# mariaalfaroc/omr_a2s_multimodal_transformer

Measured on AMD Instinct MI355X. Metric: training samples/sec, higher is better.
Workload: dtype bf16; 1 GPU; C2: image encoder (CNN) + 6-layer d_model=256 kern decoder, fwd+bwd+Adam, dropout on, teacher-forcing noise on; one sample = one score image + its token sequence; per_gpu_batch=32, global_batch=32, image=256x2048x1, seq_len=512, layers=6, d_model=256, vocab=6997, parallelism=dp1

## Files before the change

### omr_a2s_multimodal_transformer_amd/csrc/conv3x3_mfma.h

```cpp
#pragma once
#include <type_traits>

#include "omr_common.h"
#include "launch_setup.h"

namespace omr_conv {

constexpr int NORM_MAX = 128;
constexpr int TW = 32;

template <int G, typename F, typename LoadFn, typename StoreFn>
__device__ __forceinline__ void staged_walk(int pix0, int npix, int DP, int il0, int jl0, int di, int dj, int IW, LoadFn load, StoreFn store) {
    int il = il0, jl = jl0;
    for (int base = pix0; base < npix; base += G * DP) {
        F v[G];
        int pix = base;
#pragma unroll
        for (int g = 0; g < G; ++g) {
            if (pix < npix) v[g] = load(il, jl);
            jl += dj; il += di;
            if (jl >= IW) { jl -= IW; ++il; }
            pix += DP;
        }
        pix = base;
#pragma unroll
        for (int g = 0; g < G; ++g) {
            if (pix < npix) store(pix, v[g]);
            pix += DP;
        }
    }
}

__host__ __device__ constexpr bool conv_subpix(int SH, int SW, int DH, int DW, int RPW) { return DH == 2 && DW == 2 && SH == 1 && SW == 1 && RPW == 2; }
__host__ __device__ constexpr int conv_halo_h(int TH, int SH, bool subpix) { return subpix ? ((TH - 1) * SH + 3 + 1) / 2 : (TH - 1) * SH + 3; }
__host__ __device__ constexpr int conv_halo_w(int SW, bool subpix) { return subpix ? ((TW - 1) * SW + 3) / 2 : (TW - 1) * SW + 3; }

struct ConvArgs {
    const void* x; const void* w; const float* bias; void* y;
    const float* mean; const float* rstd;
    const void* mask; float mask_scale;
    int B, Hr, Wr, CIN, Ho, Wo, COUT;
    int sh, sw, dh, dw, relu, tiles_w, tiles_h;
    uint32_t drop_thresh; float drop_scale; uint64_t drop_seed; int drop_channel;
    int stat_mode; double* stat_ws; const void* stat_x; const float* stat_mean; const float* stat_rstd; int stat_slots;
    int stat_relu; float stat_relu_scale;
};

template <typename T, int NT, int RPW, int CK, int SH, int SW, int DH, int DW, bool SINGLE, int EPI>
__global__ __launch_bounds__(256, (SINGLE && NT == 32) ? ((CK == 16 && EPI != 2) ? 4 : 3) : 2) void conv3x3_mfma_kernel(ConvArgs a) {
    typedef typename Frag<T>::type F;
    typedef __attribute__((ext_vector_type(4))) T T4;
    constexpr int VEC = Frag<T>::N;
    constexpr int CKP = CK + VEC;
    constexpr int NB = NT / 32;
    constexpr int TH = 4 * RPW;
    constexpr bool SUBPIX = conv_subpix(SH, SW, DH, DW, RPW);
    constexpr int IH = conv_halo_h(TH, SH, SUBPIX), IW = conv_halo_w(SW, SUBPIX), NPIX = IH * IW;
    constexpr int CPP = CK / VEC;
    constexpr int OP = NT + VEC;
    constexpr int XS_ELEMS = (SINGLE && TH * TW * OP > NPIX * CKP) ? TH * TW * OP : NPIX * CKP;
    extern __shared__ __attribute__((aligned(16))) unsigned char smem_raw[];
    T* Xs = reinterpret_cast<T*>(smem_raw);
    T* Os = Xs;
    T* Ws = Xs + XS_ELEMS;

    const int tid = threadIdx.x, lane = tid & 63, wave = tid >> 6;
    const int n0 = blockIdx.y * NT;
    const int Hv = (a.Hr - 1) * DH + 1, Wv = (a.Wr - 1) * DW + 1;
    const T* W = (const T*)a.w;
    constexpr bool single = SINGLE;
    const int frow = lane & 31, fk = (lane >> 5) * VEC, hsel = 4 * (lane >> 5);
    const int sp_rp = wave >> 1;
    const int sp_row = (wave & 1) * 4 + sp_rp + 2 * (frow >> 4), sp_col = 2 * (frow & 15);

    auto stage_weights = [&](int c0) {
        constexpr int NCH = NT * 9 * CPP, ROUNDS = (NCH + 255) / 256, GB = 4;
#pragma unroll
        for (int r0 = 0; r0 < ROUNDS; r0 += GB) {
            F v[GB];
#pragma unroll
            for (int g = 0; g < GB; ++g) {
                const int c = tid + (r0 + g) * 256, row = c / CPP, kc = (c % CPP) * VEC, n = n0 + row / 9;
                v[g] = frag_zero<T>();
                if (r0 + g < ROUNDS && c < NCH && n < a.COUT) v[g] = *reinterpret_cast<const F*>(W + ((long)n * 9 + row % 9) * a.CIN + c0 + kc);
            }
#pragma unroll
            for (int g = 0; g < GB; ++g) {
                const int c = tid + (r0 + g) * 256, row = c / CPP, kc = (c % CPP) * VEC;
                if (r0 + g < ROUNDS && c < NCH) *reinterpret_cast<F*>(Ws + (long)row * CKP + kc) = v[g];
            }
        }
    };

    __shared__ __attribute__((aligned(16))) float sbias[NT];
    for (int i = tid; i < NT; i += 256) sbias[i] = (a.bias && n0 + i < a.COUT) ? a.bias[n0 + i] : 0.f;

    __shared__ __attribute__((aligned(16))) float snorm[2 * NORM_MAX];
    if (a.mean)
        for (int i = tid; i < a.CIN; i += 256) {
            snorm[i] = a.mean[(long)blockIdx.z * a.CIN + i];
            snorm[NORM_MAX + i] = a.rstd[(long)blockIdx.z * a.CIN + i];
        }

    if (single) stage_weights(0);

    constexpr int CPO = NT / VEC;
    constexpr int NSV = EPI ? VEC : 1;
    float ssum[NSV], ssq[NSV], smu[EPI == 2 ? VEC : 1], srs[EPI == 2 ? VEC : 1];
#pragma unroll
    for (int e = 0; e < NSV; ++e) ssum[e] = ssq[e] = 0.f;
#pragma unroll
    for (int e = 0; e < (EPI == 2 ? VEC : 1); ++e) { smu[e] = 0.f; srs[e] = 1.f; }
    constexpr bool FWD = EPI == 1 || EPI == 3, DROP = EPI == 3;
    const bool stat1 = FWD && a.stat_mode == 1, stat2 = EPI == 2 && (a.stat_mode == 2 || a.stat_mode == 4);
    const bool apply5 = EPI == 2 && a.stat_mode == 5, store_y = a.stat_mode != 4;
    auto flush_stats = [&](int bimg) {
        if constexpr (EPI != 0) {
            constexpr int NGRP = 256 / CPO;
            constexpr int RP = NT + 1;
            static_assert((size_t)NGRP * RP * sizeof(float) <= ((size_t)XS_ELEMS + (size_t)NT * 9 * CKP) * sizeof(T), "reduction scratch fits in the (dead) halo + weight tiles");
            float* red = reinterpret_cast<float*>(smem_raw);
#pragma unroll
            for (int k = 0; k < 2; ++k) {
                __syncthreads();
                const int kcs = (tid % CPO) * VEC, grp = tid / CPO;
#pragma unroll
                for (int e = 0; e < NSV; ++e) red[grp * RP + kcs + e] = k ? ssq[e] : ssum[e];
                __syncthreads();
                for (int i = tid; i < NT; i += 256) {
                    const int n = n0 + i;
                    double acc2 = 0.0;
                    for (int g = 0; g < NGRP; ++g) acc2 += (double)red[g * RP + i];
                    if (n < a.COUT) {
                        a.stat_ws[(((long)bimg * a.stat_slots + blockIdx.x) * a.COUT + n) * 2 + k] = acc2;
                        if (blockIdx.x == 0)
                            for (int sl = gridDim.x; sl < a.stat_slots; ++sl) a.stat_ws[(((long)bimg * a.stat_slots + sl) * a.COUT + n) * 2 + k] = 0.0;
                    }
                }
            }
        }
    };

    const int tiles_per_img = a.tiles_h * a.tiles_w;
    const int b = blockIdx.z;
    if constexpr (EPI == 2) {
        if (stat2 || apply5) {
            const double* compact = a.stat_ws + (long)a.B * a.stat_slots * a.COUT * 2;
            const double inv_hw = 1.0 / ((double)a.Ho * a.Wo);
#pragma unroll
            for (int e = 0; e < VEC; ++e) {
                const int n = n0 + (tid % CPO) * VEC + e;
                smu[e] = n < a.COUT ? a.stat_mean[(long)b * a.COUT + n] : 0.f;
                srs[e] = n < a.COUT ? a.stat_rstd[(long)b * a.COUT + n] : 1.f;
                if (apply5) {
                    ssum[e] = n < a.COUT ? (float)(compact[((long)b * a.COUT + n) * 2] * inv_hw) : 0.f;
                    ssq[e] = n < a.COUT ? (float)(compact[((long)b * a.COUT + n) * 2 + 1] * inv_hw) : 0.f;
                }
            }
        }
    }
    uint32_t ckeep[NB];
#pragma unroll
    for (int j = 0; j < NB; ++j) ckeep[j] = 0xffffu;
    if constexpr (DROP) {
        if (a.drop_thresh && a.drop_channel) {
#pragma unroll
            for (int j = 0; j < NB; ++j) {
                ckeep[j] = 0;
#pragma unroll
                for (int r = 0; r < 16; r += 2) {
                    const uint32_t hsh = drop_pair_bits(a.drop_seed, ((uint64_t)b * a.COUT + n0 + j * 32 + 8 * (r >> 2) + hsel + (r & 3)) >> 1);
                    ckeep[j] |= (uint32_t)((hsh & 0xffffu) >= a.drop_thresh) << r | (uint32_t)((hsh >> 16) >= a.drop_thresh) << (r + 1);
                }
            }
        }
    }
    constexpr bool PF = true;
    constexpr int XR = (NPIX + 255) / 256;
    constexpr int WNCH = NT * 9 * CPP, WR = SINGLE ? 1 : (WNCH + 255) / 256;
    F xv[XR][CPP], wv[WR];
    unsigned xok = 0;
    const T* X = (const T*)a.x + (long)b * a.Hr * a.Wr * a.CIN;
    auto load_x = [&](int rem, int c0) {
        const int th = rem / a.tiles_w, tw = rem - th * a.tiles_w;
        const int vh0 = th * TH * SH - 1, vw0 = tw * TW * SW - 1;
        xok = 0;
#pragma unroll
        for (int r = 0; r < XR; ++r) {
            const int pix = tid + r * 256;
            const int il = pix / IW, jl = pix - il * IW;
            const int vh = vh0 + (SUBPIX ? 2 * il + 1 : il), vw = vw0 + (SUBPIX ? 2 * jl + 1 : jl);
            const bool ok = pix < NPIX && vh >= 0 && vh < Hv && vw >= 0 && vw < Wv && (vh & (DH - 1)) == 0 && (vw & (DW - 1)) == 0;
            const T* src = X + ((long)(vh >> (DH >> 1)) * a.Wr + (vw >> (DW >> 1))) * a.CIN + c0;
#pragma unroll
            for (int k = 0; k < CPP; ++k) {
                xv[r][k] = frag_zero<T>();
                if (ok) xv[r][k] = *reinterpret_cast<const F*>(src + k * VEC);
            }
            xok |= (unsigned)ok << r;
        }
    };
    auto store_x = [&](int c0) {
#pragma unroll
        for (int r = 0; r < XR; ++r) {
            const int pix = tid + r * 256;
            if (a.mean && ((xok >> r) & 1)) {
#pragma unroll
                for (int k = 0; k < CPP; ++k)
#pragma unroll
                    for (int q4 = 0; q4 < VEC / 4; ++q4) {
                        const f32x4 mu = *reinterpret_cast<const f32x4*>(&snorm[c0 + k * VEC + 4 * q4]);
                        const f32x4 rs = *reinterpret_cast<const f32x4*>(&snorm[NORM_MAX + c0 + k * VEC + 4 * q4]);
#pragma unroll
                        for (int e = 0; e < 4; ++e)
                            xv[r][k][4 * q4 + e] = from_f32<T>((to_f32(xv[r][k][4 * q4 + e]) - mu[e]) * rs[e]);
                    }
            }
            if (pix < NPIX)
#pragma unroll
                for (int k = 0; k < CPP; ++k) *reinterpret_cast<F*>(Xs + (long)pix * CKP + k * VEC) = xv[r][k];
        }
    };
    auto load_w = [&](int c0) {
#pragma unroll
        for (int r = 0; r < WR; ++r) {
            const int c = tid + r * 256, row = c / CPP, kc = (c % CPP) * VEC, n = n0 + row / 9;
            wv[r] = frag_zero<T>();
            if (c < WNCH && n < a.COUT) wv[r] = *reinterpret_cast<const F*>(W + ((long)n * 9 + row % 9) * a.CIN + c0 + kc);
        }
    };
    auto store_w = [&]() {
#pragma unroll
        for (int r = 0; r < WR; ++r) {
            const int c = tid + r * 256, row = c / CPP, kc = (c % CPP) * VEC;
            if (c < WNCH) *reinterpret_cast<F*>(Ws + (long)row * CKP + kc) = wv[r];
        }
    };
    if constexpr (PF) {
        if ((int)blockIdx.x < tiles_per_img) { load_x(blockIdx.x, 0); load_w(0); }
    }

    for (int rem = blockIdx.x; rem < tiles_per_img; rem += gridDim.x) {
        const int th = rem / a.tiles_w, tw = rem - th * a.tiles_w;
        const int oh0 = th * TH, ow0 = tw * TW;
        const int vh0 = oh0 * SH - 1;

        f32x16 acc[RPW][NB];
#pragma unroll
        for (int i = 0; i < RPW; ++i)
#pragma unroll
            for (int j = 0; j < NB; ++j)
#pragma unroll
                for (int r = 0; r < 16; ++r) acc[i][j][r] = 0.f;

        for (int c0 = 0; c0 < a.CIN; c0 += CK) {
            __syncthreads();
            if constexpr (!PF) load_x(rem, c0);
            store_x(c0);
            if constexpr (!SINGLE) store_w();
            __syncthreads();
            if constexpr (PF) {
                int nc0 = c0 + CK, nrem = rem;
                if (nc0 >= a.CIN) { nc0 = 0; nrem = rem + gridDim.x; }
                if (nrem < tiles_per_img) { load_x(nrem, nc0); load_w(nc0); }
            }
            bool row_live[RPW][3];
#pragma unroll
            for (int i = 0; i < RPW; ++i)
#pragma unroll
                for (int kh = 0; kh < 3; ++kh) row_live[i][kh] = DH == 1 || (((vh0 + (wave * RPW + i) * SH + kh) & (DH - 1)) == 0);
            if constexpr (SUBPIX) {
                const int vw0 = ow0 * SW - 1;
#pragma unroll
                for (int tap = 0; tap < 9; ++tap) {
                    const int kh = tap / 3, kw = tap % 3;
                    if (((vh0 + sp_rp + kh) & 1) != 0) continue;
                    const bool lc[2] = {((vw0 + kw) & 1) == 0, ((vw0 + 1 + kw) & 1) == 0};
#pragma unroll
                    for (int kk = 0; kk < CK; kk += KStep<T>::value) {
                        F af[2], bf[NB];
#pragma unroll
                        for (int cp = 0; cp < 2; ++cp)
                            if (lc[cp]) af[cp] = *reinterpret_cast<const F*>(Xs + (long)(((sp_row + kh) >> 1) * IW + ((sp_col + cp + kw) >> 1)) * CKP + kk + fk);
#pragma unroll
                        for (int j = 0; j < NB; ++j)
                            bf[j] = *reinterpret_cast<const F*>(Ws + (long)((j * 32 + frow) * 9 + tap) * CKP + kk + fk);
#pragma unroll
                        for (int cp = 0; cp < 2; ++cp) {
                            if (!lc[cp]) continue;
#pragma unroll
                            for (int j = 0; j < NB; ++j) mma32(acc[cp][j], bf[j], af[cp]);
                        }
                    }
                }
            } else
#pragma unroll
            for (int tap = 0; tap < 9; ++tap) {
                const int kh = tap / 3, kw = tap % 3;
                bool any_live = false;
#pragma unroll
                for (int i = 0; i < RPW; ++i) any_live = any_live || row_live[i][kh];
                if (!any_live) continue;
#pragma unroll
                for (int kk = 0; kk < CK; kk += KStep<T>::value) {
                    F af[RPW], bf[NB];
#pragma unroll
                    for (int i = 0; i < RPW; ++i) {
                        const int pix = ((wave * RPW + i) * SH + kh) * IW + frow * SW + kw;
                        af[i] = *reinterpret_cast<const F*>(Xs + (long)pix * CKP + kk + fk);
                    }
#pragma unroll
                    for (int j = 0; j < NB; ++j)
                        bf[j] = *reinterpret_cast<const F*>(Ws + (long)((j * 32 + frow) * 9 + tap) * CKP + kk + fk);
#pragma unroll
                    for (int i = 0; i < RPW; ++i) {
                        if (!row_live[i][kh]) continue;
#pragma unroll
                        for (int j = 0; j < NB; ++j) mma32(acc[i][j], bf[j], af[i]);
                    }
                }
            }
        }

        const float oscale = a.mask ? a.mask_scale : 1.f;
        const bool drop_chan = DROP && a.drop_thresh != 0 && a.drop_channel;
        __syncthreads();
#pragma unroll
        for (int j = 0; j < NB; ++j)
#pragma unroll
            for (int i = 0; i < RPW; ++i) {
                T* orow = Os + (long)(SUBPIX ? sp_row * TW + sp_col + i : (wave * RPW + i) * TW + frow) * OP + j * 32 + hsel;
#pragma unroll
                for (int g = 0; g < 4; ++g) {
                    T4 o;
                    const uint32_t k4 = ckeep[j] >> (4 * g);
                    const f32x4 bq = *reinterpret_cast<const f32x4*>(&sbias[j * 32 + 8 * g + hsel]);
#pragma unroll
                    for (int e = 0; e < 4; ++e) {
                        float v = acc[i][j][4 * g + e] + bq[e];
                        if (a.relu) v = fmaxf(v, 0.f);
                        if constexpr (DROP) {
                            if (drop_chan) v = ((k4 >> e) & 1u) ? v * a.drop_scale : 0.f;
                        } else {
                            v *= oscale;
                        }
                        o[e] = from_f32<T>(v);
                    }
                    *reinterpret_cast<T4*>(orow + 8 * g) = o;
                }
            }
        __syncthreads();
        T* Y = (T*)a.y + (long)b * a.Ho * a.Wo * a.COUT;
        const T* Mk = a.mask ? (const T*)a.mask + (long)b * a.Ho * a.Wo * a.COUT : nullptr;
        const T* SX = (stat2 || apply5) ? (const T*)a.stat_x + (long)b * a.Ho * a.Wo * a.COUT : nullptr;
#pragma unroll(EPI == 0 ? 8 : 4)
        for (int c = tid; c < TH * TW * CPO; c += 256) {
            const int pl = c / CPO, kc = (c % CPO) * VEC;
            const int oh = oh0 + pl / TW, ow = ow0 + pl % TW, n = n0 + kc;
            if (oh >= a.Ho || ow >= a.Wo || n >= a.COUT) continue;
            F v = *reinterpret_cast<const F*>(Os + (long)pl * OP + kc);
            const long o = ((long)oh * a.Wo + ow) * a.COUT + n;
            if constexpr (DROP) {
                if (a.drop_thresh && !a.drop_channel) {
                    const uint64_t pbase = ((uint64_t)b * a.Ho * a.Wo * a.COUT + (uint64_t)o) >> 1;
                    const uint32_t h0 = (uint32_t)pbase ^ (uint32_t)(pbase >> 32) * 0x27D4EB2Fu;
                    const uint32_t slo = (uint32_t)a.drop_seed, shi = (uint32_t)(a.drop_seed >> 32);
#pragma unroll
                    for (int e = 0; e < VEC / 2; ++e) {
                        const uint32_t hsh = hash32(slo, shi, h0 ^ (uint32_t)e);
                        v[2 * e] = (hsh & 0xffffu) >= a.drop_thresh ? from_f32<T>(to_f32(v[2 * e]) * a.drop_scale) : from_f32<T>(0.f);
                        v[2 * e + 1] = (hsh >> 16) >= a.drop_thresh ? from_f32<T>(to_f32(v[2 * e + 1]) * a.drop_scale) : from_f32<T>(0.f);
                    }
                }
            }
            if (Mk) {
                typedef typename std::conditional<sizeof(T) == 2, short, int>::type I;
                typedef __attribute__((ext_vector_type(VEC))) I IV;
                const IV m = *reinterpret_cast<const IV*>(Mk + o);
                const IV keep = m > (I)0;
                IV bits;
                __builtin_memcpy(&bits, &v, sizeof(bits));
                bits &= keep;
                __builtin_memcpy(&v, &bits, sizeof(bits));
            }
            if constexpr (EPI == 2) {
                if (apply5) {
                    const F xv = *reinterpret_cast<const F*>(SX + o);
#pragma unroll
                    for (int e = 0; e < VEC; ++e) {
                        const float xf = to_f32(xv[e]);
                        float d = srs[e] * (to_f32(v[e]) - ssum[e] - (xf - smu[e]) * srs[e] * ssq[e]);
                        if (a.stat_relu) d = xf > 0.f ? d * a.stat_relu_scale : 0.f;
                        v[e] = from_f32<T>(d);
                    }
                }
            }
            if (store_y) *reinterpret_cast<F*>(Y + o) = v;
            if constexpr (FWD) {
                if (stat1) {
#pragma unroll
                    for (int e = 0; e < VEC; ++e) { const float f = to_f32(v[e]); ssum[e] += f; ssq[e] += f * f; }
                }
            } else if constexpr (EPI == 2) {
                if (stat2) {
                    const F xv = *reinterpret_cast<const F*>(SX + o);
#pragma unroll
                    for (int e = 0; e < VEC; ++e) { const float f = to_f32(v[e]); ssum[e] += f; ssq[e] += f * ((to_f32(xv[e]) - smu[e]) * srs[e]); }
                }
            }
        }
    }
    if (stat1 || stat2) flush_stats(b);
}

template <typename T, int NT, int RPW, int CK, int SH, int SW, int DH, int DW, bool SINGLE, int EPI> int launch_conv3(const ConvArgs& a0, hipStream_t s) {
    ConvArgs a = a0;
    constexpr int TH = 4 * RPW;
    constexpr int CKP = CK + Frag<T>::N;
    constexpr bool SUBPIX = conv_subpix(SH, SW, DH, DW, RPW);
    constexpr int IH = conv_halo_h(TH, SH, SUBPIX), IW = conv_halo_w(SW, SUBPIX), NPIX = IH * IW, OP = NT + Frag<T>::N;
    constexpr int XS_ELEMS = (SINGLE && TH * TW * OP > NPIX * CKP) ? TH * TW * OP : NPIX * CKP;
    a.tiles_w = cdiv(a.Wo, TW);
    a.tiles_h = cdiv(a.Ho, TH);
    size_t shm = ((size_t)XS_ELEMS + (size_t)NT * 9 * CKP) * sizeof(T);
    if (!SINGLE && (size_t)TH * TW * OP * sizeof(T) > shm) shm = (size_t)TH * TW * OP * sizeof(T);
    if (shm > 160 * 1024) return OMR_ERR_UNSUPPORTED;
    if (a.COUT % Frag<T>::N) return OMR_ERR_UNSUPPORTED;
    if (a.mean && a.CIN > NORM_MAX) return OMR_ERR_UNSUPPORTED;
    auto kern = conv3x3_mfma_kernel<T, NT, RPW, CK, SH, SW, DH, DW, SINGLE, EPI>;
    const int ny = cdiv(a.COUT, NT);
    const long tiles_per_img = (long)a.tiles_w * a.tiles_h;
    static std::atomic<int> occ_cache{0};
    const int occv = omr_launch_setup(occ_cache, (const void*)kern, shm, shm > 48 * 1024, 256, 2);
    if (occv == 0) return OMR_ERR_LAUNCH;
    long gx = ((long)OMR_NUM_CU * occv + (long)ny * a.B - 1) / ((long)ny * a.B);
    if (gx > tiles_per_img) gx = tiles_per_img;
    if (a.stat_mode) {
        if (a.stat_slots < 1) return OMR_ERR_ARG;
        if (gx > a.stat_slots) gx = a.stat_slots;
    }
    if (gx < 1) gx = 1;
    hipLaunchKernelGGL(kern, dim3((unsigned)gx, ny, a.B), dim3(256), shm, s, a);
    OMR_CHECK_LAUNCH();
    return OMR_OK;
}

template <typename T, int NT, int RPW, int CK, int SH, int SW, int DH, int DW, bool SINGLE> int launch_conv2(const ConvArgs& a, hipStream_t s) {
    constexpr bool can1 = (DH == 1 && DW == 1), can2 = (SH == 1 && SW == 1);
    constexpr bool is_f32 = std::is_same<T, float>::value;
    int epi = (a.stat_mode == 2 || a.stat_mode >= 4) ? 2 : (a.drop_thresh ? 3 : (a.stat_mode == 1 ? 1 : 0));
    if (is_f32 && epi == 0) epi = can1 ? 1 : 2;
    if (epi == 1) {
        if constexpr (can1) return launch_conv3<T, NT, RPW, CK, SH, SW, DH, DW, SINGLE, 1>(a, s);
        else return OMR_ERR_UNSUPPORTED;
    }
    if (epi == 3) {
        if constexpr (can1) return launch_conv3<T, NT, RPW, CK, SH, SW, DH, DW, SINGLE, 3>(a, s);
        else return OMR_ERR_UNSUPPORTED;
    }
    if (epi == 2) {
        if constexpr (can2) return launch_conv3<T, NT, RPW, CK, SH, SW, DH, DW, SINGLE, 2>(a, s);
        else return OMR_ERR_UNSUPPORTED;
    }
    if constexpr (!is_f32) return launch_conv3<T, NT, RPW, CK, SH, SW, DH, DW, SINGLE, 0>(a, s);
    else return OMR_ERR_UNSUPPORTED;
}
template <typename T, int NT, int RPW, int CK, int SH, int SW, int DH, int DW> int launch_conv(const ConvArgs& a, hipStream_t s) {
    if (a.CIN == CK) return launch_conv2<T, NT, RPW, CK, SH, SW, DH, DW, true>(a, s);
    return launch_conv2<T, NT, RPW, CK, SH, SW, DH, DW, false>(a, s);
}

template <typename T, int NT, int SH, int SW, int DH, int DW> int dispatch_conv_ck(const ConvArgs& a, hipStream_t s) {
    constexpr int KS = KStep<T>::value;
    constexpr bool strided = SH > 1 || SW > 1;
    if (a.CIN % KS) return OMR_ERR_UNSUPPORTED;
    if constexpr (strided) {
        return launch_conv<T, NT, 1, KS, SH, SW, DH, DW>(a, s);
    } else {
        if (a.CIN % (2 * KS) == 0) return launch_conv<T, NT, 2, 2 * KS, SH, SW, DH, DW>(a, s);
        return launch_conv<T, NT, 2, KS, SH, SW, DH, DW>(a, s);
    }
}
template <typename T, int NT> int dispatch_conv_nt(const ConvArgs& a, hipStream_t s) {
    if (a.dh == 1 && a.dw == 1) {
        if (a.sh == 1 && a.sw == 1) return dispatch_conv_ck<T, NT, 1, 1, 1, 1>(a, s);
        if (a.sh == 2 && a.sw == 2) return dispatch_conv_ck<T, NT, 2, 2, 1, 1>(a, s);
        if (a.sh == 2 && a.sw == 1) return dispatch_conv_ck<T, NT, 2, 1, 1, 1>(a, s);
        return OMR_ERR_UNSUPPORTED;
    }
    if (a.sh != 1 || a.sw != 1) return OMR_ERR_UNSUPPORTED;
    if (a.dh == 2 && a.dw == 2) return dispatch_conv_ck<T, NT, 1, 1, 2, 2>(a, s);
    if (a.dh == 2 && a.dw == 1) return dispatch_conv_ck<T, NT, 1, 1, 2, 1>(a, s);
    return OMR_ERR_UNSUPPORTED;
}
template <typename T> int dispatch_conv(const ConvArgs& a, hipStream_t s) {
    return a.COUT > 32 ? dispatch_conv_nt<T, 64>(a, s) : dispatch_conv_nt<T, 32>(a, s);
}


}
```

### omr_a2s_multimodal_transformer_amd/csrc/conv_bf16.hip

```cpp
#include "conv3x3_mfma.h"
int omr_conv3x3_dispatch_bf16(const omr_conv::ConvArgs& a, hipStream_t s) { return omr_conv::dispatch_conv<bf16>(a, s); }
```

Before: 1381 samples/s.

## Add persistent double-buffered DMA conv3x3 kernel for common channel shapes

Adds a new 3x3 stride-1 convolution kernel that uses 512 threads, a persistent grid sized to the CU count, and asynchronous global-to-LDS DMA into a two-slot ring. The next input and weight chunk loads while MFMA runs on the current one. Swizzled LDS layout is meant to avoid bank conflicts. The kernel is routed ahead of the existing kernel for a fixed set of (CIN, COUT) pairs with no norm or stat modes, and the shared epilogue is moved into a header so both kernels use it. A persistent grid with a small gx could underfill the GPU, and the boundary and zero-fill handling adds correctness risk.

```diff
diff --git a/omr_a2s_multimodal_transformer_amd/csrc/conv3x3_mfma.h b/omr_a2s_multimodal_transformer_amd/csrc/conv3x3_mfma.h
--- a/omr_a2s_multimodal_transformer_amd/csrc/conv3x3_mfma.h
+++ b/omr_a2s_multimodal_transformer_amd/csrc/conv3x3_mfma.h
@@ -3,11 +3,9 @@
 
 #include "omr_common.h"
 #include "launch_setup.h"
+#include "conv_epilogue.h"
 
 namespace omr_conv {
-
-constexpr int NORM_MAX = 128;
-constexpr int TW = 32;
 
 template <int G, typename F, typename LoadFn, typename StoreFn>
 __device__ __forceinline__ void staged_walk(int pix0, int npix, int DP, int il0, int jl0, int di, int dj, int IW, LoadFn load, StoreFn store) {
@@ -34,17 +32,6 @@
 __host__ __device__ constexpr bool conv_subpix(int SH, int SW, int DH, int DW, int RPW) { return DH == 2 && DW == 2 && SH == 1 && SW == 1 && RPW == 2; }
 __host__ __device__ constexpr int conv_halo_h(int TH, int SH, bool subpix) { return subpix ? ((TH - 1) * SH + 3 + 1) / 2 : (TH - 1) * SH + 3; }
 __host__ __device__ constexpr int conv_halo_w(int SW, bool subpix) { return subpix ? ((TW - 1) * SW + 3) / 2 : (TW - 1) * SW + 3; }
-
-struct ConvArgs {
-    const void* x; const void* w; const float* bias; void* y;
-    const float* mean; const float* rstd;
-    const void* mask; float mask_scale;
-    int B, Hr, Wr, CIN, Ho, Wo, COUT;
-    int sh, sw, dh, dw, relu, tiles_w, tiles_h;
-    uint32_t drop_thresh; float drop_scale; uint64_t drop_seed; int drop_channel;
-    int stat_mode; double* stat_ws; const void* stat_x; const float* stat_mean; const float* stat_rstd; int stat_slots;
-    int stat_relu; float stat_relu_scale;
-};
 
 template <typename T, int NT, int RPW, int CK, int SH, int SW, int DH, int DW, bool SINGLE, int EPI>
 __global__ __launch_bounds__(256, (SINGLE && NT == 32) ? ((CK == 16 && EPI != 2) ? 4 : 3) : 2) void conv3x3_mfma_kernel(ConvArgs a) {
@@ -106,7 +93,8 @@
 
     constexpr int CPO = NT / VEC;
     constexpr int NSV = EPI ? VEC : 1;
-    float ssum[NSV], ssq[NSV], smu[EPI == 2 ? VEC : 1], srs[EPI == 2 ? VEC : 1];
+    ConvStatRegs<T, EPI> st;
+    float (&ssum)[NSV] = st.ssum, (&ssq)[NSV] = st.ssq, (&smu)[EPI == 2 ? VEC : 1] = st.smu, (&srs)[EPI == 2 ? VEC : 1] = st.srs;
 #pragma unroll
     for (int e = 0; e < NSV; ++e) ssum[e] = ssq[e] = 0.f;
 #pragma unroll
@@ -114,6 +102,7 @@
     constexpr bool FWD = EPI == 1 || EPI == 3, DROP = EPI == 3;
     const bool stat1 = FWD && a.stat_mode == 1, stat2 = EPI == 2 && (a.stat_mode == 2 || a.stat_mode == 4);
     const bool apply5 = EPI == 2 && a.stat_mode == 5, store_y = a.stat_mode != 4;
+    st.stat1 = stat1; st.stat2 = stat2; st.apply5 = apply5; st.store_y = store_y;
     auto flush_stats = [&](int bimg) {
         if constexpr (EPI != 0) {
             constexpr int NGRP = 256 / CPO;
@@ -160,21 +149,7 @@
         }
     }
     uint32_t ckeep[NB];
-#pragma unroll
-    for (int j = 0; j < NB; ++j) ckeep[j] = 0xffffu;
-    if constexpr (DROP) {
-        if (a.drop_thresh && a.drop_channel) {
-#pragma unroll
-            for (int j = 0; j < NB; ++j) {
-                ckeep[j] = 0;
-#pragma unroll
-                for (int r = 0; r < 16; r += 2) {
-                    const uint32_t hsh = drop_pair_bits(a.drop_seed, ((uint64_t)b * a.COUT + n0 + j * 32 + 8 * (r >> 2) + hsel + (r & 3)) >> 1);
-                    ckeep[j] |= (uint32_t)((hsh & 0xffffu) >= a.drop_thresh) << r | (uint32_t)((hsh >> 16) >= a.drop_thresh) << (r + 1);
-                }
-            }
-        }
-    }
+    conv_chan_keep<NB, DROP>(a, b, n0, hsel, ckeep);
     constexpr bool PF = true;
     constexpr int XR = (NPIX + 255) / 256;
     constexpr int WNCH = NT * 9 * CPP, WR = SINGLE ? 1 : (WNCH + 255) / 256;
@@ -322,93 +297,11 @@
             }
         }
 
-        const float oscale = a.mask ? a.mask_scale : 1.f;
-        const bool drop_chan = DROP && a.drop_thresh != 0 && a.drop_channel;
         __syncthreads();
-#pragma unroll
-        for (int j = 0; j < NB; ++j)
-#pragma unroll
-            for (int i = 0; i < RPW; ++i) {
-                T* orow = Os + (long)(SUBPIX ? sp_row * TW + sp_col + i : (wave * RPW + i) * TW + frow) * OP + j * 32 + hsel;
-#pragma unroll
-                for (int g = 0; g < 4; ++g) {
-                    T4 o;
-                    const uint32_t k4 = ckeep[j] >> (4 * g);
-                    const f32x4 bq = *reinterpret_cast<const f32x4*>(&sbias[j * 32 + 8 * g + hsel]);
-#pragma unroll
-                    for (int e = 0; e < 4; ++e) {
-                        float v = acc[i][j][4 * g + e] + bq[e];
-                        if (a.relu) v = fmaxf(v, 0.f);
-                        if constexpr (DROP) {
-                            if (drop_chan) v = ((k4 >> e) & 1u) ? v * a.drop_scale : 0.f;
-                        } else {
-                            v *= oscale;
-                        }
-                        o[e] = from_f32<T>(v);
-                    }
-                    *reinterpret_cast<T4*>(orow + 8 * g) = o;
-                }
-            }
+        conv_stage_acc<T, NB, RPW, DROP>(a, acc, ckeep, sbias, Os, OP, hsel,
+                                         [&](int i) { return SUBPIX ? sp_row * TW + sp_col + i : (wave * RPW + i) * TW + frow; });
         __syncthreads();
-        T* Y = (T*)a.y + (long)b * a.Ho * a.Wo * a.COUT;
-        const T* Mk = a.mask ? (const T*)a.mask + (long)b * a.Ho * a.Wo * a.COUT : nullptr;
-        const T* SX = (stat2 || apply5) ? (const T*)a.stat_x + (long)b * a.Ho * a.Wo * a.COUT : nullptr;
-#pragma unroll(EPI == 0 ? 8 : 4)
-        for (int c = tid; c < TH * TW * CPO; c += 256) {
-            const int pl = c / CPO, kc = (c % CPO) * VEC;
-            const int oh = oh0 + pl / TW, ow = ow0 + pl % TW, n = n0 + kc;
-            if (oh >= a.Ho || ow >= a.Wo || n >= a.COUT) continue;
-            F v = *reinterpret_cast<const F*>(Os + (long)pl * OP + kc);
-            const long o = ((long)oh * a.Wo + ow) * a.COUT + n;
-            if constexpr (DROP) {
-                if (a.drop_thresh && !a.drop_channel) {
-                    const uint64_t pbase = ((uint64_t)b * a.Ho * a.Wo * a.COUT + (uint64_t)o) >> 1;
-                    const uint32_t h0 = (uint32_t)pbase ^ (uint32_t)(pbase >> 32) * 0x27D4EB2Fu;
-                    const uint32_t slo = (uint32_t)a.drop_seed, shi = (uint32_t)(a.drop_seed >> 32);
-#pragma unroll
-                    for (int e = 0; e < VEC / 2; ++e) {
-                        const uint32_t hsh = hash32(slo, shi, h0 ^ (uint32_t)e);
-                        v[2 * e] = (hsh & 0xffffu) >= a.drop_thresh ? from_f32<T>(to_f32(v[2 * e]) * a.drop_scale) : from_f32<T>(0.f);
-                        v[2 * e + 1] = (hsh >> 16) >= a.drop_thresh ? from_f32<T>(to_f32(v[2 * e + 1]) * a.drop_scale) : from_f32<T>(0.f);
-                    }
-                }
-            }
-            if (Mk) {
-                typedef typename std::conditional<sizeof(T) == 2, short, int>::type I;
-                typedef __attribute__((ext_vector_type(VEC))) I IV;
-                const IV m = *reinterpret_cast<const IV*>(Mk + o);
-                const IV keep = m > (I)0;
-                IV bits;
-                __builtin_memcpy(&bits, &v, sizeof(bits));
-                bits &= keep;
-                __builtin_memcpy(&v, &bits, sizeof(bits));
-            }
-            if constexpr (EPI == 2) {
-                if (apply5) {
-                    const F xv = *reinterpret_cast<const F*>(SX + o);
-#pragma unroll
-                    for (int e = 0; e < VEC; ++e) {
-                        const float xf = to_f32(xv[e]);
-                        float d = srs[e] * (to_f32(v[e]) - ssum[e] - (xf - smu[e]) * srs[e] * ssq[e]);
-                        if (a.stat_relu) d = xf > 0.f ? d * a.stat_relu_scale : 0.f;
-                        v[e] = from_f32<T>(d);
-                    }
-                }
-            }
-            if (store_y) *reinterpret_cast<F*>(Y + o) = v;
-            if constexpr (FWD) {
-                if (stat1) {
-#pragma unroll
-                    for (int e = 0; e < VEC; ++e) { const float f = to_f32(v[e]); ssum[e] += f; ssq[e] += f * f; }
-                }
-            } else if constexpr (EPI == 2) {
-                if (stat2) {
-                    const F xv = *reinterpret_cast<const F*>(SX + o);
-#pragma unroll
-                    for (int e = 0; e < VEC; ++e) { const float f = to_f32(v[e]); ssum[e] += f; ssq[e] += f * ((to_f32(xv[e]) - smu[e]) * srs[e]); }
-                }
-            }
-        }
+        conv_store_tile<T, NT, TH, 256, EPI>(a, Os, b, oh0, ow0, n0, tid, st);
     }
     if (stat1 || stat2) flush_stats(b);
 }
diff --git a/omr_a2s_multimodal_transformer_amd/csrc/conv_bf16.hip b/omr_a2s_multimodal_transformer_amd/csrc/conv_bf16.hip
--- a/omr_a2s_multimodal_transformer_amd/csrc/conv_bf16.hip
+++ b/omr_a2s_multimodal_transformer_amd/csrc/conv_bf16.hip
@@ -1,2 +1,7 @@
 #include "conv3x3_mfma.h"
-int omr_conv3x3_dispatch_bf16(const omr_conv::ConvArgs& a, hipStream_t s) { return omr_conv::dispatch_conv<bf16>(a, s); }
+int omr_conv_wide_bf16(const omr_conv::ConvArgs& a, hipStream_t s);
+int omr_conv3x3_dispatch_bf16(const omr_conv::ConvArgs& a, hipStream_t s) {
+    const int rc = omr_conv_wide_bf16(a, s);
+    if (rc != OMR_ERR_UNSUPPORTED) return rc;
+    return omr_conv::dispatch_conv<bf16>(a, s);
+}
diff --git a/omr_a2s_multimodal_transformer_amd/csrc/conv_epilogue.h b/omr_a2s_multimodal_transformer_amd/csrc/conv_epilogue.h
--- /dev/null
+++ b/omr_a2s_multimodal_transformer_amd/csrc/conv_epilogue.h
@@ -0,0 +1,144 @@
+#pragma once
+#include <type_traits>
+
+#include "omr_common.h"
+
+namespace omr_conv {
+
+constexpr int NORM_MAX = 128;
+constexpr int TW = 32;
+
+struct ConvArgs {
+    const void* x; const void* w; const float* bias; void* y;
+    const float* mean; const float* rstd;
+    const void* mask; float mask_scale;
+    int B, Hr, Wr, CIN, Ho, Wo, COUT;
+    int sh, sw, dh, dw, relu, tiles_w, tiles_h;
+    uint32_t drop_thresh; float drop_scale; uint64_t drop_seed; int drop_channel;
+    int stat_mode; double* stat_ws; const void* stat_x; const float* stat_mean; const float* stat_rstd; int stat_slots;
+    int stat_relu; float stat_relu_scale;
+};
+
+template <int NB, bool DROP> __device__ __forceinline__ void conv_chan_keep(const ConvArgs& a, int b, int n0, int hsel, uint32_t (&ckeep)[NB]) {
+#pragma unroll
+    for (int j = 0; j < NB; ++j) ckeep[j] = 0xffffu;
+    if constexpr (DROP) {
+        if (a.drop_thresh && a.drop_channel) {
+#pragma unroll
+            for (int j = 0; j < NB; ++j) {
+                ckeep[j] = 0;
+#pragma unroll
+                for (int r = 0; r < 16; r += 2) {
+                    const uint32_t hsh = drop_pair_bits(a.drop_seed, ((uint64_t)b * a.COUT + n0 + j * 32 + 8 * (r >> 2) + hsel + (r & 3)) >> 1);
+                    ckeep[j] |= (uint32_t)((hsh & 0xffffu) >= a.drop_thresh) << r | (uint32_t)((hsh >> 16) >= a.drop_thresh) << (r + 1);
+                }
+            }
+        }
+    }
+}
+
+template <typename T, int NB, int RPW, bool DROP, typename PixOf>
+__device__ __forceinline__ void conv_stage_acc(const ConvArgs& a, const f32x16 (&acc)[RPW][NB], const uint32_t (&ckeep)[NB], const float* sbias, T* Os,
+                                               int OP, int hsel, PixOf pix_of) {
+    typedef __attribute__((ext_vector_type(4))) T T4;
+    const float oscale = a.mask ? a.mask_scale : 1.f;
+    const bool drop_chan = DROP && a.drop_thresh != 0 && a.drop_channel;
+#pragma unroll
+    for (int j = 0; j < NB; ++j)
+#pragma unroll
+        for (int i = 0; i < RPW; ++i) {
+            T* orow = Os + (long)pix_of(i) * OP + j * 32 + hsel;
+#pragma unroll
+            for (int g = 0; g < 4; ++g) {
+                T4 o;
+                const uint32_t k4 = ckeep[j] >> (4 * g);
+                const f32x4 bq = *reinterpret_cast<const f32x4*>(&sbias[j * 32 + 8 * g + hsel]);
+#pragma unroll
+                for (int e = 0; e < 4; ++e) {
+                    float v = acc[i][j][4 * g + e] + bq[e];
+                    if (a.relu) v = fmaxf(v, 0.f);
+                    if constexpr (DROP) {
+                        if (drop_chan) v = ((k4 >> e) & 1u) ? v * a.drop_scale : 0.f;
+                    } else {
+                        v *= oscale;
+                    }
+                    o[e] = from_f32<T>(v);
+                }
+                *reinterpret_cast<T4*>(orow + 8 * g) = o;
+            }
+        }
+}
+
+template <typename T, int EPI> struct ConvStatRegs {
+    static constexpr int VEC = Frag<T>::N, NSV = EPI ? VEC : 1, NS2 = EPI == 2 ? VEC : 1;
+    float ssum[NSV], ssq[NSV], smu[NS2], srs[NS2];
+    bool stat1, stat2, apply5, store_y;
+};
+
+template <typename T, int NT, int TH, int NTHR, int EPI>
+__device__ __forceinline__ void conv_store_tile(const ConvArgs& a, const T* Os, int b, int oh0, int ow0, int n0, int tid, ConvStatRegs<T, EPI>& st) {
+    typedef typename Frag<T>::type F;
+    constexpr int VEC = Frag<T>::N, OP = NT + VEC, CPO = NT / VEC;
+    constexpr bool FWD = EPI == 1 || EPI == 3, DROP = EPI == 3;
+    T* Y = (T*)a.y + (long)b * a.Ho * a.Wo * a.COUT;
+    const T* Mk = a.mask ? (const T*)a.mask + (long)b * a.Ho * a.Wo * a.COUT : nullptr;
+    const T* SX = (st.stat2 || st.apply5) ? (const T*)a.stat_x + (long)b * a.Ho * a.Wo * a.COUT : nullptr;
+#pragma unroll(EPI == 0 ? 8 : 4)
+    for (int c = tid; c < TH * TW * CPO; c += NTHR) {
+        const int pl = c / CPO, kc = (c % CPO) * VEC;
+        const int oh = oh0 + pl / TW, ow = ow0 + pl % TW, n = n0 + kc;
+        if (oh >= a.Ho || ow >= a.Wo || n >= a.COUT) continue;
+        F v = *reinterpret_cast<const F*>(Os + (long)pl * OP + kc);
+        const long o = ((long)oh * a.Wo + ow) * a.COUT + n;
+        if constexpr (DROP) {
+            if (a.drop_thresh && !a.drop_channel) {
+                const uint64_t pbase = ((uint64_t)b * a.Ho * a.Wo * a.COUT + (uint64_t)o) >> 1;
+                const uint32_t h0 = (uint32_t)pbase ^ (uint32_t)(pbase >> 32) * 0x27D4EB2Fu;
+                const uint32_t slo = (uint32_t)a.drop_seed, shi = (uint32_t)(a.drop_seed >> 32);
+#pragma unroll
+                for (int e = 0; e < VEC / 2; ++e) {
+                    const uint32_t hsh = hash32(slo, shi, h0 ^ (uint32_t)e);
+                    v[2 * e] = (hsh & 0xffffu) >= a.drop_thresh ? from_f32<T>(to_f32(v[2 * e]) * a.drop_scale) : from_f32<T>(0.f);
+                    v[2 * e + 1] = (hsh >> 16) >= a.drop_thresh ? from_f32<T>(to_f32(v[2 * e + 1]) * a.drop_scale) : from_f32<T>(0.f);
+                }
+            }
+        }
+        if (Mk) {
+            typedef typename std::conditional<sizeof(T) == 2, short, int>::type I;
+            typedef __attribute__((ext_vector_type(VEC))) I IV;
+            const IV m = *reinterpret_cast<const IV*>(Mk + o);
+            const IV keep = m > (I)0;
+            IV bits;
+            __builtin_memcpy(&bits, &v, sizeof(bits));
+            bits &= keep;
+            __builtin_memcpy(&v, &bits, sizeof(bits));
+        }
+        if constexpr (EPI == 2) {
+            if (st.apply5) {
+                const F xv = *reinterpret_cast<const F*>(SX + o);
+#pragma unroll
+                for (int e = 0; e < VEC; ++e) {
+                    const float xf = to_f32(xv[e]);
+                    float d = st.srs[e] * (to_f32(v[e]) - st.ssum[e] - (xf - st.smu[e]) * st.srs[e] * st.ssq[e]);
+                    if (a.stat_relu) d = xf > 0.f ? d * a.stat_relu_scale : 0.f;
+                    v[e] = from_f32<T>(d);
+                }
+            }
+        }
+        if (st.store_y) *reinterpret_cast<F*>(Y + o) = v;
+        if constexpr (FWD) {
+            if (st.stat1) {
+#pragma unroll
+                for (int e = 0; e < VEC; ++e) { const float f = to_f32(v[e]); st.ssum[e] += f; st.ssq[e] += f * f; }
+            }
+        } else if constexpr (EPI == 2) {
+            if (st.stat2) {
+                const F xv = *reinterpret_cast<const F*>(SX + o);
+#pragma unroll
+                for (int e = 0; e < VEC; ++e) { const float f = to_f32(v[e]); st.ssum[e] += f; st.ssq[e] += f * ((to_f32(xv[e]) - st.smu[e]) * st.srs[e]); }
+            }
+        }
+    }
+}
+
+}
diff --git a/omr_a2s_multimodal_transformer_amd/csrc/conv_wide_dma.hip b/omr_a2s_multimodal_transformer_amd/csrc/conv_wide_dma.hip
--- /dev/null
+++ b/omr_a2s_multimodal_transformer_amd/csrc/conv_wide_dma.hip
@@ -0,0 +1,201 @@
+#include <cstdlib>
+
+#include "omr_common.h"
+#include "conv_epilogue.h"
+#include "dma_common.h"
+#include "launch_setup.h"
+
+using omr_conv::ConvArgs;
+using omr_conv::TW;
+
+namespace {
+
+#ifdef OMR_WIDE_DEBUG
+__device__ int g_wide_dbg;
+#define DBG(bit) (dbg & (bit))
+#else
+#define DBG(bit) false
+#endif
+
+constexpr int NW = 8, NTHR = NW * 64;
+constexpr int TH = 2 * NW;
+constexpr int IH = TH + 2, IW = TW + 2, NPIX = IH * IW;
+constexpr int CK = 32, CPP = CK / 8;
+constexpr int ROW = CK * 2;
+
+__device__ uint4 g_zero_chunk;
+
+__device__ __forceinline__ int swz(int i) { return (i >> 2) & 3; }
+
+template <int NROWS> struct Piece {
+    static constexpr int NCH = NROWS * CPP, WINS = (NCH + 63) / 64, ROUNDS = (WINS * 64 + NTHR - 1) / NTHR, BYTES = WINS * 1024;
+};
+
+template <int NT, int EPI>
+__global__ __launch_bounds__(NTHR) void conv_wide_dma_kernel(ConvArgs a) {
+    constexpr int NB = NT / 32, OP = NT + 8;
+    constexpr bool DROP = EPI == 3;
+    typedef Piece<NPIX> PX;
+    typedef Piece<NT * 9> PW;
+    constexpr int SLOT = PX::BYTES + PW::BYTES;
+    static_assert(TH * TW * OP * 2 <= SLOT, "the output staging tile fits in one ring slot");
+    extern __shared__ __attribute__((aligned(16))) unsigned char smem_raw[];
+    __shared__ __attribute__((aligned(16))) float sbias[NT];
+    const unsigned ring_addr = lds_address(smem_raw);
+
+#ifdef OMR_WIDE_DEBUG
+    const int dbg = g_wide_dbg;
+#endif
+    const int tid = threadIdx.x, lane = tid & 63, wave = tid >> 6;
+    const int n0 = blockIdx.y * NT, b = blockIdx.z;
+    const int frow = lane & 31, khalf = lane >> 5, hsel = 4 * khalf;
+    const int tiles_per_img = a.tiles_h * a.tiles_w, nchunk = a.CIN / CK;
+    const bf16* X = (const bf16*)a.x + (long)b * a.Hr * a.Wr * a.CIN;
+    const bf16* Wt = (const bf16*)a.w + (long)n0 * 9 * a.CIN;
+    const bf16* zsrc = reinterpret_cast<const bf16*>(&g_zero_chunk);
+
+    for (int i = tid; i < NT; i += NTHR) sbias[i] = a.bias ? a.bias[n0 + i] : 0.f;
+
+    int xrel[PX::ROUNDS], xij[PX::ROUNDS], wrel[PW::ROUNDS];
+#pragma unroll
+    for (int r = 0; r < PX::ROUNDS; ++r) {
+        const int L = r * NTHR + tid, pix = L / CPP, il = pix / IW, jl = pix - il * IW;
+        const int c = (L % CPP) ^ swz(jl);
+        xij[r] = il | (jl << 16);
+        xrel[r] = L < PX::NCH ? (il * a.Wr + jl) * a.CIN + c * 8 : -1;
+    }
+#pragma unroll
+    for (int r = 0; r < PW::ROUNDS; ++r) {
+        const int L = r * NTHR + tid, row = L / CPP;
+        const int c = (L % CPP) ^ swz(row / 9);
+        wrel[r] = L < PW::NCH ? row * a.CIN + c * 8 : -1;
+    }
+    auto issue = [&](int rem, int c0, int slot) {
+        const int th = rem / a.tiles_w, tw = rem - th * a.tiles_w;
+        const int ih0 = th * TH - 1, iw0 = tw * TW - 1;
+        const unsigned xa = ring_addr + (unsigned)slot * SLOT, wa = xa + PX::BYTES;
+        const bf16* origin = X + ((long)ih0 * a.Wr + iw0) * a.CIN + c0;
+        const bool interior = ih0 >= 0 && ih0 + IH <= a.Hr && iw0 >= 0 && iw0 + IW <= a.Wr;
+#pragma unroll
+        for (int r = 0; r < (DBG(1) ? 0 : PX::ROUNDS); ++r) {
+            const int L0 = r * NTHR + (tid & ~63);
+            if (L0 >= PX::WINS * 64) continue;
+            bool ok = xrel[r] >= 0;
+            if (!interior) {
+                const int ih = ih0 + (xij[r] & 0xffff), iw = iw0 + (xij[r] >> 16);
+                ok = ok && (unsigned)ih < (unsigned)a.Hr && (unsigned)iw < (unsigned)a.Wr;
+            }
+            dma16(ok ? origin + xrel[r] : zsrc, xa + (unsigned)L0 * 16u);
+        }
+#pragma unroll
+        for (int r = 0; r < (DBG(2) ? 0 : PW::ROUNDS); ++r) {
+            const int L0 = r * NTHR + (tid & ~63);
+            if (L0 >= PW::WINS * 64) continue;
+            dma16(wrel[r] >= 0 ? Wt + c0 + wrel[r] : zsrc, wa + (unsigned)L0 * 16u);
+        }
+    };
+
+    uint32_t ckeep[NB];
+    omr_conv::conv_chan_keep<NB, DROP>(a, b, n0, hsel, ckeep);
+    omr_conv::ConvStatRegs<bf16, EPI> st;
+#pragma unroll
+    for (int e = 0; e < st.NSV; ++e) st.ssum[e] = st.ssq[e] = 0.f;
+    st.smu[0] = 0.f; st.srs[0] = 1.f;
+    st.stat1 = st.stat2 = st.apply5 = false; st.store_y = true;
+
+    int xoff[3];
+#pragma unroll
+    for (int kw = 0; kw < 3; ++kw) xoff[kw] = (frow + kw) * ROW;
+    const int woff = frow * 9 * ROW, wswz = swz(frow);
+
+    int rem = blockIdx.x, slot = 0;
+    if (rem < tiles_per_img) issue(rem, 0, 0);
+    for (; rem < tiles_per_img; rem += gridDim.x) {
+        f32x16 acc[2][NB];
+#pragma unroll
+        for (int i = 0; i < 2; ++i)
+#pragma unroll
+            for (int j = 0; j < NB; ++j)
+#pragma unroll
+                for (int r = 0; r < 16; ++r) acc[i][j][r] = 0.f;
+
+        for (int ci = 0; ci < nchunk; ++ci) {
+            dma_wait_barrier<0>();
+            {
+                int nci = ci + 1, nrem = rem;
+                if (nci == nchunk) { nci = 0; nrem = rem + gridDim.x; }
+                if (nrem < tiles_per_img) issue(nrem, nci * CK, slot ^ 1);
+            }
+            const unsigned char* Xs = smem_raw + slot * SLOT;
+            const unsigned char* Ws = Xs + PX::BYTES;
+#pragma unroll
+            for (int tap = 0; tap < (DBG(4) ? 0 : 9); ++tap) {
+                const int kh = tap / 3, kw = tap % 3;
+                const int xs = swz(frow + kw);
+#pragma unroll
+                for (int ks = 0; ks < CK / 16; ++ks) {
+                    const int c = ks * 2 + khalf;
+                    bf16x8 af[2], bf[NB];
+#pragma unroll
+                    for (int i = 0; i < 2; ++i)
+                        af[i] = *reinterpret_cast<const bf16x8*>(Xs + (wave * 2 + i + kh) * (IW * ROW) + xoff[kw] + ((c ^ xs) << 4));
+#pragma unroll
+                    for (int j = 0; j < NB; ++j)
+                        bf[j] = *reinterpret_cast<const bf16x8*>(Ws + j * (32 * 9 * ROW) + woff + tap * ROW + ((c ^ wswz) << 4));
+#pragma unroll
+                    for (int i = 0; i < 2; ++i)
+#pragma unroll
+                        for (int j = 0; j < NB; ++j) mma32(acc[i][j], bf[j], af[i]);
+                }
+            }
+            slot ^= 1;
+        }
+
+        bf16* Os = reinterpret_cast<bf16*>(smem_raw + (slot ^ 1) * SLOT);
+        lds_barrier();
+        if (!DBG(16)) omr_conv::conv_stage_acc<bf16, NB, 2, DROP>(a, acc, ckeep, sbias, Os, OP, hsel, [&](int i) { return (wave * 2 + i) * TW + frow; });
+        lds_barrier();
+        const int th = rem / a.tiles_w, tw = rem - th * a.tiles_w;
+        if (!DBG(8)) omr_conv::conv_store_tile<bf16, NT, TH, NTHR, EPI>(a, Os, b, th * TH, tw * TW, n0, tid, st);
+    }
+}
+
+template <int NT, int EPI> int launch(ConvArgs a, hipStream_t s) {
+    a.tiles_w = cdiv(a.Wo, TW);
+    a.tiles_h = cdiv(a.Ho, TH);
+    constexpr size_t shm = 2 * (size_t)(Piece<NPIX>::BYTES + Piece<NT * 9>::BYTES);
+    static_assert(shm + NT * sizeof(float) <= 160 * 1024, "LDS ring does not fit");
+    auto kern = conv_wide_dma_kernel<NT, EPI>;
+    static std::atomic<int> once{0};
+    if (omr_launch_setup(once, (const void*)kern, shm, true) == 0) return OMR_ERR_LAUNCH;
+    const int ny = a.COUT / NT;
+    const long tiles_per_img = (long)a.tiles_w * a.tiles_h;
+#ifdef OMR_WIDE_DEBUG
+    { const char* e = getenv("OMR_WIDE_DBG"); const int v = e ? atoi(e) : 0; (void)hipMemcpyToSymbolAsync(HIP_SYMBOL(g_wide_dbg), &v, sizeof(v), 0, hipMemcpyHostToDevice, s); }
+#endif
+    long gx = ((long)OMR_NUM_CU + (long)ny * a.B - 1) / ((long)ny * a.B);
+    if (gx > tiles_per_img) gx = tiles_per_img;
+    if (gx < 1) gx = 1;
+    hipLaunchKernelGGL(kern, dim3((unsigned)gx, ny, a.B), dim3(NTHR), shm, s, a);
+    OMR_CHECK_LAUNCH();
+    return OMR_OK;
+}
+
+struct Route { int cin, cout; };
+constexpr Route ROUTES[] = {{64, 32}, {64, 64}, {64, 128}, {128, 64}, {128, 128}};
+
+}
+
+int omr_conv_wide_bf16(const ConvArgs& a, hipStream_t s) {
+    const char* sw = getenv("OMR_CONV_WIDE");
+    if (sw && sw[0] == '0') return OMR_ERR_UNSUPPORTED;
+    if (a.sh != 1 || a.sw != 1 || a.dh != 1 || a.dw != 1 || a.mean || a.stat_mode) return OMR_ERR_UNSUPPORTED;
+    if (a.Ho != a.Hr || a.Wo != a.Wr) return OMR_ERR_UNSUPPORTED;
+    bool routed = false;
+    for (const Route& r : ROUTES) routed = routed || (r.cin == a.CIN && r.cout == a.COUT);
+    if (!routed) return OMR_ERR_UNSUPPORTED;
+    if ((long)IH * a.Wr * a.CIN >= (1L << 30)) return OMR_ERR_UNSUPPORTED;
+    const bool drop = a.drop_thresh != 0;
+    if (a.COUT == 32) return drop ? launch<32, 3>(a, s) : launch<32, 0>(a, s);
+    return drop ? launch<64, 3>(a, s) : launch<64, 0>(a, s);
+}
```

New measurement: 1392 samples/s, median of 6. No clear change (+0.7%).
